# AbnerVictor/OOD-GAN-inversion

Hardware: AMD Instinct MI355X
Metric: 1024² face inversions/sec (100 W+ steps) (higher is better)
Workload: dtype f16-split (hi+lo f16 operands, f32 accumulate): 3 MFMA/product in every forward conv (fp32-equivalent), 2 in the input-gradient convs (back-propagated gradient rounded to f16 before each contraction, weights keep hi+lo); dL/dW+ vs the float64 reference 1.4e-5..3.6e-5 ('f16s': 1.3e-5..2.6e-5, the ref

## Files before the change

include/oodgan.h:

```cpp
#ifndef OODGAN_H
#define OODGAN_H

#ifdef __cplusplus
extern "C" {
#endif

#define OODGAN_OK 0
#define OODGAN_E_ARG (-1)
#define OODGAN_E_LAUNCH (-2)
#define OODGAN_E_STATE (-3)
#define OODGAN_E_NODEV (-4)

int oodgan_version(void);
const char* oodgan_last_error(void);
int oodgan_device_count(void);
int oodgan_set_tunable(const char* name, long value);
long oodgan_get_tunable(const char* name);
long oodgan_dispatch_count(const char* name);
int oodgan_dispatch_reset(void);
int oodgan_zero(void* p, long bytes, void* stream);

void* oodgan_plan_create(void);
int oodgan_plan_destroy(void* plan);
int oodgan_plan_record_begin(void* plan);
// ... 227 lines not shown
int oodgan_reduce_parts(const float* part, float* out, long rows, int nparts, int accumulate, void* stream);
int oodgan_reduce_parts_cols(const float* part, float* out, int B, int C, int nparts, int out_stride, int accumulate,
                             void* stream);


int oodgan_torgb_fwd(const float* x, const float* w, const float* s, int s_stride, const float* bias,
                     const float* skip, const float* kernel, float* y, int B, int Ci, int H, int W,
                     float scale, void* stream);
int oodgan_torgb_fwd_sform(const float* x, const float* w, const float* s, int s_stride, const float* bias,
                           const float* skip, const float* kernel, float* y, void* ys, const float* ys_scale,
                           int ys_scale_stride, int B, int Ci, int H, int W, float scale, unsigned* vmax, void* stream);
int oodgan_rgb_finish(const float* partial, const float* bias, const float* skip, const float* kernel, float* y, int B, int H,
                      int W, void* stream);
int oodgan_rgb_finish_parts(const float* partial, int nparts, const float* bias, const float* skip, const float* kernel, float* y, int B,
                            int H, int W, void* stream);

int oodgan_feature_modulation(const float* x, const float* c0, const float* c1, float* y, long n, int mode, void* stream);

int oodgan_act_bwd_fused(const float* g_feat, const float* out, const float* noise, int noise_batch,
                         const float* noise_w, const float* bias, const float* g_rgb, const float* w_rgb,
                         const float* s_rgb, int s_rgb_stride, float rgb_scale, float* g_pre,
                         float* part_r, float* part_rgb, int B, int C, long HW, void* stream);
int oodgan_act_bwd_nparts(long HW);
int oodgan_act_bwd_fused_max(const float* g_feat, const float* out, const float* noise, int noise_batch,
                             const float* noise_w, const float* bias, const float* g_rgb, const float* w_rgb,
                             const float* s_rgb, int s_rgb_stride, float rgb_scale, float* g_pre,
                             float* part_r, float* part_rgb, float* part_max, const float* dscale, int dscale_stride, int B,
                             int C, long HW, void* stream);
int oodgan_absmax_scale(const float* part, long n, float* out2, void* stream);
int oodgan_absmax_scale_clear(float* part, long n, float* out2, void* stream);
// ... 138 lines not shown
```

ood-gan-inversion_amd/csrc/common.hpp:

```cpp
#pragma once
#include <hip/hip_runtime.h>
#include <cstdio>
#include <cstdarg>
#include <functional>
#include <utility>
#include "../../include/oodgan.h"

namespace oodgan {
struct PlanRec;
extern thread_local PlanRec* tl_plan_rec;
extern int g_null_launch;
void plan_append(std::function<void()>&& f);
template <class F>
inline void launch_rec(F&& f) {
    f();
    if (__builtin_expect(tl_plan_rec != nullptr, 0)) plan_append(std::function<void()>(std::forward<F>(f)));
}
}
#undef hipLaunchKernelGGL
#define hipLaunchKernelGGL(kernelName, numBlocks, numThreads, memPerBlock, streamId, ...)                                        \
    ::oodgan::launch_rec([=]() {                                                                                                 \
        if (!::oodgan::g_null_launch) (kernelName)<<<(numBlocks), (numThreads), (memPerBlock), (streamId)>>>(__VA_ARGS__);      \
    })

namespace oodgan {

void set_error(const char* fmt, ...);

enum { OODGAN_TUN_S1_BIG_MIN_ITEMS = 0, OODGAN_TUN_S2_BIG_MIN_ITEMS, OODGAN_TUN_T2_BIG_MIN_ITEMS, OODGAN_TUN_BLURT_STRIP, OODGAN_TUN_BLUR_STRIP, OODGAN_TUN_UPVB_WAVES, OODGAN_TUN_FEWOUT_QUAD, OODGAN_TUN_TINY_MID_MAX, OODGAN_TUN_STRIPX_WAVES, OODGAN_TUN_BLURT_SEG_ROWS, OODGAN_TUN_COUNT };
long tunable(int id);

enum { OODGAN_DC_STRIPX = 0, OODGAN_DC_STRIP, OODGAN_DC_S1BIG, OODGAN_DC_S1V2, OODGAN_DC_S1PP, OODGAN_DC_TINY, OODGAN_DC_T2BIG,
       OODGAN_DC_T2V2, OODGAN_DC_T2GEN, OODGAN_DC_S2BIG, OODGAN_DC_S2V2, OODGAN_DC_S2GEN, OODGAN_DC_UPVB,
       OODGAN_DC_S1BIG_YS, OODGAN_DC_S2BIG_FUSE, OODGAN_DC_S2BIG_DOTXS,
       OODGAN_DC_S1BIG_G2, OODGAN_DC_S2BIG_G2, OODGAN_DC_STRIPX_G2, OODGAN_DC_S2BIG_XH, OODGAN_DC_S1BIG_XH,
       OODGAN_DC_COMPOSITE_MSE,
       OODGAN_DC_SSIM,
       OODGAN_DC_ROBUST,
       OODGAN_DC_AREA_POOL,
       OODGAN_DC_POOLED_PIXEL,
       OODGAN_DC_PN,
       OODGAN_DC_RESAMPLED_PIXEL,
       OODGAN_DC_BLURT_STRIP, OODGAN_DC_BLURT_TILE, OODGAN_DC_ACTBWD_SFORM, OODGAN_DC_ACTBWD_SFORM_F, OODGAN_DC_COUNT };
void count_dispatch(int id);

bool bound_device_ok(const char* what);

inline int check_launch(const char* what) {
    hipError_t e = hipGetLastError();
    if (e != hipSuccess) {
        set_error("%s: %s", what, hipGetErrorString(e));
        return OODGAN_E_LAUNCH;
    }
    return OODGAN_OK;
}

#define OODGAN_REQUIRE(cond, ...)          \
    do {                                    \
// ... 146 lines not shown
```

ood-gan-inversion_amd/csrc/runtime.hip:

```cpp
#include "common.hpp"
#include <atomic>
#include <cstdlib>
#include <cstring>
#include <new>

namespace oodgan {
static thread_local char g_err[512] = "";
void set_error(const char* fmt, ...) {
    va_list ap;
    va_start(ap, fmt);
    vsnprintf(g_err, sizeof(g_err), fmt, ap);
    va_end(ap);
}
}

namespace oodgan {
namespace {
struct Tunable { const char* name; const char* env; long def; std::atomic<long> val; std::atomic<int> init; };
Tunable g_tun[OODGAN_TUN_COUNT] = {
    {"s1_big_min_items", "OODGAN_S1_BIG_MIN_ITEMS", 128, {0}, {0}},
    {"s2_big_min_items", "OODGAN_S2_BIG_MIN_ITEMS", 128, {0}, {0}},
    {"t2_big_min_items", "OODGAN_T2_BIG_MIN_ITEMS", 128, {0}, {0}},
    {"blurt_strip", "OODGAN_BLURT_STRIP", 1, {0}, {0}},
    {"blur_strip", "OODGAN_BLUR_STRIP", 1, {0}, {0}},
    {"upvb_waves", "OODGAN_UPVB_WAVES", 12, {0}, {0}},
    {"fewout_quad", "OODGAN_FEWOUT_QUAD", 1, {0}, {0}},
    {"tiny_mid_max", "OODGAN_TINY_MID_MAX", 1024, {0}, {0}},
    {"stripx_waves", "OODGAN_STRIPX_WAVES", 4, {0}, {0}},
    {"blurt_seg_rows", "OODGAN_BLURT_SEG_ROWS", 0, {0}, {0}},
};
}
long tunable(int id) {
    Tunable& t = g_tun[id];
    if (!t.init.load(std::memory_order_acquire)) {
        const char* e = getenv(t.env);
        t.val.store(e ? atol(e) : t.def, std::memory_order_relaxed);
        t.init.store(1, std::memory_order_release);
    }
    return t.val.load(std::memory_order_relaxed);
}
}

extern "C" int oodgan_set_tunable(const char* name, long value) {
    OODGAN_REQUIRE(name != nullptr, "set_tunable: null name");
// ... 20 lines not shown
    if (hipGetDevice(&dev) != hipSuccess) {
        (void)hipGetLastError();
        set_error("%s: no current HIP device", what);
        return false;
    }
    int expected = -1;
    if (bound.compare_exchange_strong(expected, dev, std::memory_order_acq_rel) || expected == dev) return true;
    set_error("%s: liboodgan_hip.so is bound to HIP device %d (its first use in this process) but device %d is current — one process per GPU "
              "(select the device with HIP_VISIBLE_DEVICES or torch.cuda.set_device before the first call)", what, expected, dev);
    return false;
}
}

namespace oodgan {
namespace {
const char* const g_dc_name[OODGAN_DC_COUNT] = {"stripx", "strip", "s1big", "s1v2", "s1pp", "tiny", "t2big", "t2v2", "t2gen", "s2big", "s2v2", "s2gen", "upvb", "s1big_ys", "s2big_fuse", "s2big_dotx_sform", "s1big_g2", "s2big_g2", "stripx_g2", "s2big_xh", "s1big_xh", "composite_mse", "ssim", "robust", "area_pool", "pooled_pixel", "pn", "resampled_pixel", "blurt_strip", "blurt_tile", "actbwd_sform", "actbwd_sform_f"};
std::atomic<long> g_dc[OODGAN_DC_COUNT];
}
void count_dispatch(int id) { g_dc[id].fetch_add(1, std::memory_order_relaxed); }
}
extern "C" long oodgan_dispatch_count(const char* name) {
    if (name)
        for (int i = 0; i < oodgan::OODGAN_DC_COUNT; ++i)
            if (strcmp(name, oodgan::g_dc_name[i]) == 0) return oodgan::g_dc[i].load(std::memory_order_relaxed);
    return -1;
}
extern "C" int oodgan_dispatch_reset(void) {
    for (int i = 0; i < oodgan::OODGAN_DC_COUNT; ++i) oodgan::g_dc[i].store(0, std::memory_order_relaxed);
    return OODGAN_OK;
}

// ... 85 lines not shown
```

ood-gan-inversion_amd/oodgan/_lib.py:

```python
import ctypes
import os
from ctypes import POINTER, Structure, c_char_p, c_double, c_float, c_int, c_long, c_void_p

_HERE = os.path.dirname(os.path.abspath(__file__))
LIB_PATH = os.environ.get('OODGAN_LIB') or os.path.join(_HERE, 'liboodgan_hip.so')

CONV_S1, CONV_T2, CONV_S2 = 0, 1, 2
ACT_NONE, ACT_LRELU, ACT_PRELU = 0, 1, 2

P = c_void_p


ABI_VERSION = 117


class ConvArgs(Structure):
    _fields_ = [
        ('x', P), ('wpk', P), ('in_scale', P), ('in_shift', P), ('out_scale', P), ('bias', P), ('noise', P),
        ('noise_w', P), ('slope', P), ('dotx', P), ('dot_part', P), ('y', P),
        ('B', c_int), ('K', c_int), ('M', c_int), ('Hin', c_int), ('Win', c_int),
        ('in_pitch', c_int), ('out_pitch', c_int), ('in_scale_stride', c_int), ('out_scale_stride', c_int),
        ('noise_batch', c_int), ('mode', c_int), ('act', c_int), ('dot_nparts', c_int), ('in_mul2', P),
        ('x_sform', c_int), ('ys', P), ('ys_scale', P), ('ys_scale_stride', c_int),
        ('rgb_w', P), ('rgb_s', P), ('rgb_y', P), ('rgb_s_stride', c_int), ('rgb_scale', c_float), ('fuse', P), ('dot_actgrad', c_int), ('groups', c_int), ('y_fform', c_int), ('x_fform', c_int), ('dotx_fform', c_int), ('dotx_sform', c_int), ('dotx_scale', P), ('dotx_scale_stride', c_int), ('workspace', P), ('workspace_bytes', c_long), ('ys_vmax', P), ('x_hi_only', c_int),
# ... 95 lines not shown
    'oodgan_demod_bwd_batch': (c_int, [P, c_int, P]),
    'oodgan_demod_fwd_batch': (c_int, [P, c_int, P]),
    'oodgan_absmax_scale_check_batch': (c_int, [P, c_int, P, P]),
    'oodgan_hform_bytes': (c_long, [c_int, c_int, c_int, c_int]),
    'oodgan_to_hform': (c_int, [P, P, c_int, c_int, c_int, c_int, P]),
    'oodgan_from_hform': (c_int, [P, P, c_int, c_int, c_int, c_int, P]),
    'oodgan_modconv_f16_wbytes': (c_long, [c_int, c_int, c_int]),
    'oodgan_modconv_f16_pack': (c_int, [P, P, c_int, c_float, c_int, c_int, P, c_int, c_int, c_int, P]),
    'oodgan_modconv_f16_pack_affine': (c_int, [P, P, c_int, P, P, c_int, c_float, c_int, c_int, P, c_int, c_int, c_int, P]),
    'oodgan_modconv_f16': (c_int, [P, P, P, c_int, P, P, c_int, P, c_int, c_int, c_int, c_int, c_int, P]),
    'oodgan_reduce_parts': (c_int, [P, P, c_long, c_int, c_int, P]),
    'oodgan_reduce_parts_cols': (c_int, [P, P, c_int, c_int, c_int, c_int, c_int, P]),
    'oodgan_torgb_fwd': (c_int, [P, P, P, c_int, P, P, P, P, c_int, c_int, c_int, c_int, c_float, P]),
    'oodgan_rgb_finish': (c_int, [P, P, P, P, P, c_int, c_int, c_int, P]),
    'oodgan_rgb_finish_parts': (c_int, [P, c_int, P, P, P, P, c_int, c_int, c_int, P]),
    'oodgan_torgb_fwd_sform': (c_int, [P, P, P, c_int, P, P, P, P, P, P, c_int, c_int, c_int, c_int, c_int, c_float, P, P]),
    'oodgan_act_bwd_fused': (c_int, [P, P, P, c_int, P, P, P, P, P, c_int, c_float, P, P, P, c_int, c_int, c_long, P]),
    'oodgan_act_bwd_nparts': (c_int, [c_long]),
    'oodgan_feature_modulation': (c_int, [P, P, P, P, c_long, c_int, P]),
    'oodgan_act_bwd_fused_max': (c_int, [P, P, P, c_int, P, P, P, P, P, c_int, c_float, P, P, P, P, P, c_int, c_int, c_int, c_long, P]),
    'oodgan_absmax_scale': (c_int, [P, c_long, P, P]),
    'oodgan_absmax_scale_clear': (c_int, [P, c_long, P, P]),
    'oodgan_mse_fwd_bwd': (c_int, [P, P, P, P, P, c_int, c_long, c_float, P]),
    'oodgan_mse_fwd_bwd_row': (c_int, [P, P, P, P, P, P, c_int, c_int, c_long, c_float, P]),
    'oodgan_conv2d_s1': (c_int, [P, P, P, P, P, P, c_int, c_int, c_int, c_int, c_int, c_int, c_int, c_int, P]),
    'oodgan_add_mask': (c_int, [P, P, P, c_long, P]),
    'oodgan_maxpool3s2_fwd': (c_int, [P, P, P, c_long, c_int, c_int, P]),
    'oodgan_maxpool3s2_bwd': (c_int, [P, P, P, P, P, c_long, c_int, c_int, P]),
    'oodgan_lpips_prep': (c_int, [P, P, c_int, c_int, c_int, c_float, c_float, POINTER(c_float), POINTER(c_float), P]),
    'oodgan_lpips_img_grad': (c_int, [P, P, c_int, c_int, c_int, c_float, c_float, POINTER(c_float), P]),
# ... 117 lines not shown
```

ood-gan-inversion_amd/oodgan/engine.py:

```python
import math
import numbers
import re

import os

import torch

from . import ops
from ._lib import ACT_LRELU, ACT_NONE, CONV_S1, CONV_S2, CONV_T2
from .synth import generator_channels, make_kernel


_Cols = ops.Cols


class _Layer:
    __slots__ = ('name', 'kind', 'cin', 'cout', 'res', 'lat', 'row', 'drow', 'wpk', 'wpk_bwd', 'wsq', 'w_rgb',
                 'bias', 'noise_w', 'scale', 'noise_idx', 'src', 'sidx', 'wpk_vb')


def _pad_channels_to_16(state, prefix, log_size, ch):
    up16 = lambda c: (c + 15) // 16 * 16
    chp = {r: up16(c) for r, c in ch.items()}
    out = dict(state)
# ... 242 lines not shown
    def style_layout(self):
        if self.padded:
            raise NotImplementedError('style_layout() of a generator whose channel counts are zero-padded to multiples of 16')
        lay = style_layout(self.log_size, lambda name: self.by_name[name].cin)
        assert lay == [(L.name, L.lat, L.row, L.cin) for L in self.layers]
        return lay

    def feature_shape(self, l):
        l = check_feature_layer(l, self.n_latent)
        if self.padded:
            raise NotImplementedError('feature_layer on a generator whose channel counts are zero-padded to multiples of 16')
        L = next(L for L in self.layers if L.kind == 'up' and L.lat == l)
        return (L.cin, L.res // 2, L.res // 2)

    def forward(self, latent, noises, save=False, cond_hook=None, cond_layers=None, return_features=False, features_in=None,
                feature_scale=1.0, range_mode='exact', post_hook=None, style_offsets=None, feature_offset=None, feature_out=None):
        if self.padded and (cond_hook is not None or features_in is not None or post_hook is not None):
            raise NotImplementedError('conditioning hooks / feature injection on a generator whose channel counts are zero-padded to multiples of 16')
        if save and (features_in is not None or post_hook is not None):
            raise NotImplementedError('backward through an injected feature / feature modulation is not part of the path')
        if self.padded and style_offsets is not None:
            raise NotImplementedError('style offsets on a generator whose channel counts are zero-padded to multiples of 16')
        B = latent.shape[0]
        f_lat, f_delta, f_in = None, None, None
        if feature_offset is not None:
            f_lat, f_delta = feature_offset
            if tuple(f_delta.shape) != (B,) + self.feature_shape(f_lat):
                raise ValueError(f'feature_offset for latent {f_lat} must be {(B,) + self.feature_shape(f_lat)}, got {tuple(f_delta.shape)}')
        self._fwd_serial += 1
        s_all = self.styles(latent, style_offsets)
        d_all = torch.empty(B, self.DR, device=self.device, dtype=torch.float32)
# ... 26 lines not shown
                                vmax=rng.vm[L.sidx] if carry else None)

        acts = {}
        ck = (B, ops._stream_handle())
        x = self._const_b.get(ck)
        if x is None:
            x = self._const_b[ck] = self.const_input.expand(B, -1, -1, -1).contiguous()
        acts['input'] = x
        skip, out = None, x
        pending = None
        rgb_partial = None
        i = 1
        for L in self.layers:
            s = _Cols(s_all, L.row, L.cin)
            if L.kind == 'rgb' and rgb_partial is not None:
                skip = ops.rgb_finish(rgb_partial, L.bias, skip, self.k_up if skip is not None else None)
                rgb_partial = None
                continue
            if L.kind == 'rgb':
                Lu = self.rgb_next_up.get(L.name) if (carry and self.fused_rgb) else None
                if (Lu is not None and pending is None and out.shape[2] * out.shape[3] > 4096 and L.cin % 16 == 0
                        and out.shape[3] % 4 == 0):
                    pending = ops.sform_scratch(B, L.cin, out.shape[2], out.shape[3], self.device)
                    skip = ops.torgb(out, L.w_rgb, s, L.bias, skip, self.k_up if skip is not None else None, ys=pending,
                                     ys_scale=_Cols(s_use, Lu.row, Lu.cin), vmax=rng.vm[Lu.sidx])
                else:
                    skip = ops.torgb(out, L.w_rgb, s, L.bias, skip, self.k_up if skip is not None else None)
                continue
            d = _Cols(d_use, L.drow, L.cout)
            nz = noises[L.noise_idx]
            if features_in is not None and L.lat >= 1 and L.lat < len(features_in) and features_in[L.lat] is not None:
# ... 118 lines not shown
            return skip, (feat[:, :self.real_channels[self.size]].contiguous() if self.padded else feat)
        return skip

    def _demod(self, L, s_all, d_all):
        from ._lib import lib, check
        import ctypes
        B = s_all.shape[0]
        check(lib().oodgan_demod_fwd(ctypes.c_void_p(s_all.data_ptr() + 4 * L.row), self.R, ctypes.c_void_p(L.wsq.data_ptr()),
                                     ctypes.c_void_p(d_all.data_ptr() + 4 * L.drow), self.DR, B, L.cin, L.cout, L.scale,
                                     ops._stream()), 'demod_fwd')

    def _hi_records(self, B, L, Hd, Rg):
        return bool(self.grad_hi_only and self.hi_records and Rg is None and ops.blurT_hi_supported(Hd, Hd)
                    and ops.s2_fuse_supported(B, L.cout, L.cin, 2 * Hd + 1, 2 * Hd + 1))

    def backward(self, gimg, grad_scale=1.0, carry_scale=False, wrt='latent', feature_grad=None):
        from ._lib import lib, check
        import ctypes
        if wrt not in ('latent', 'styles'):
            raise ValueError(f"wrt must be 'latent' or 'styles', got {wrt!r}")
        sv = self.saved
        if sv is None:
            raise RuntimeError('backward() without forward(save=True)')
        if sv['serial'] != self._fwd_serial:
            raise RuntimeError('backward(): another forward of this engine ran after forward(save=True) — the saved activations (pooled S-form / F-form '
                               'buffers, scales of the range state) may have been overwritten; call backward() right after the forward it belongs to')
        acts, s_all, d_all, noises, B = sv['acts'], sv['s_all'], sv['d_all'], sv['noises'], sv['B']
        f_lat, f_in = sv['f_lat'], sv['f_in']
        if (feature_grad is not None) != (f_lat is not None):
            raise RuntimeError('backward(feature_grad=) goes with forward(feature_offset=, save=True), and one needs the other')
        if feature_grad is not None and not (tuple(feature_grad.shape) == tuple(f_in.shape) and feature_grad.dtype == torch.float32
                                             and feature_grad.is_contiguous() and feature_grad.device == f_in.device):
            raise ValueError(f'feature_grad must be a contiguous float32 {tuple(f_in.shape)} tensor on {f_in.device}')
        gs_all = ops.zeros(B, self.R, device=self.device)
        gskip = {self.size: gimg.contiguous()}
        r = self.size
        while r > 4:
            gskip[r // 2] = ops.upfirdn2d(gskip[r], self.k_up_flip, up=1, down=2, pad=(1, 1))
            r //= 2
        g_feat = None
        prev_rgb = None
        fused_in = None
        fused_pre = None
        jobs = ops.BwdJobs() if (carry_scale and self.fused_bwd and self.sform and self.batched_tail) else None
        for L in reversed(self.layers):
            if L.kind == 'rgb':
                prev_rgb = L
                continue
            out, x_in, nz = acts[L.name], acts[L.src], noises[L.noise_idx]
            at_f = L.lat == f_lat
            if at_f:
# ... 153 lines not shown
        return torch.cuda.MemPool()
    key = (str(device), ops._stream_handle(), int(batch))
    pool = _PLAN_POOLS.get(key)
    if pool is None:
        pool = _PLAN_POOLS[key] = torch.cuda.MemPool()
    return pool


def _flag_stream(device):
    st = _FLAG.get(str(device))
    if st is None:
        st = _FLAG[str(device)] = torch.cuda.Stream(device=device)
    return st


class _WRun:

    def __init__(self, inv, eng, target, w0, noises, steps, stream, keep_traj, replay, beta=None, ids=None, anchor=None, f0=None, pn=None,
                 px=None, ml0=None):
        self.inv, self.eng, self.stream, self.steps = inv, eng, stream, steps
        self.target, self.noises = target, noises
        self.beta = beta
        self.sspace = inv.latent_space == 's'
        self.w0 = w0.detach().clone().contiguous() if self.sspace else None
        self.w = torch.zeros(w0.shape[0], eng.R, device=w0.device, dtype=torch.float32) if self.sspace else w0.detach().clone().contiguous()
        self.m, self.v = torch.zeros_like(self.w), torch.zeros_like(self.w)
        self.gmul = ops.loss_scale_for(target.numel() // target.shape[0])
        self.t = 0
        self.dev_t = torch.zeros(1, dtype=torch.int32, device=self.w.device)
        self.lbuf = torch.empty(steps, self.w.shape[0], device=self.w.device, dtype=torch.float32)
# ... 25 lines not shown
            self.fm, self.fv, self.fg, self.fx = (torch.zeros_like(self.f) for _ in range(4))
            if inv.feature_reg != 0.0:
                self.ft_table = torch.zeros(steps, self.w.shape[0], device=self.w.device, dtype=torch.float32)
                self.fpart = ops.feature_step_parts(self.f.shape[0], self.f.numel() // self.f.shape[0], self.f.device)
        self.pn = pn
        self.pn_table = torch.zeros(steps, self.w.shape[0], device=self.w.device, dtype=torch.float32) if inv.pn_reg != 0.0 else None
        self.pn_part = ops.pn_prior_parts(self.w.shape[0], self.w.shape[1], self.w.device) if self.pn_table is not None else None
        self.ml = self.mm = self.mv = self.mg = self.ma = self.me = self.mstat = self.ma_table = self.mb_table = None
        if ml0 is not None:
            Bm, S = self.w.shape[0], int(target.shape[-1])
            self.ml = ml0.detach().clone().contiguous()
            self.mm, self.mv, self.mg, self.ma = (torch.zeros_like(self.ml) for _ in range(4))
            self.beta, self.me = (torch.empty(Bm, 1, S, S, device=self.w.device, dtype=torch.float32) for _ in range(2))
            self.mstat = ops.maskfit_stat(Bm, self.w.device)
            self.ma_table, self.mb_table = (torch.zeros(steps, Bm, device=self.w.device, dtype=torch.float32) for _ in range(2))
        self.traj = [None] * steps if keep_traj else None
        self.mode0 = (eng.fused_bwd, eng.carry_range)
        self.guard = (eng.fused_bwd or eng.carry_range) and inv.check_every > 0 and replay != 'graph'
        self.clean = (0, self.w.clone(), None, None, self._fsnap(), self._msnap()) if self.guard else None
        self.pending, self.exact_until = None, 0
        self.steps_run = 0
        self.rollbacks = 0
        self.host = inv._pinned(len(inv._runs)) if self.guard else None
        inv._runs.append(self)
        if replay == 'plan' and (keep_traj or not eng.sform):
            replay = None
        self.replay, self.warmup = replay, 1 if replay == 'graph' else 2
        self.plan, self.pool, self.eager_left, self.plan_steps, self.plan_size = None, None, self.warmup, 0, 0

    def _eager_step(self):
# ... 7 lines not shown
                           style_reg=inv.style_reg, table=self.st_table)
            return
        w_in = self.w
        if self.w_in is not None:
            w_in = ops.latent_noise(self.w, self.dev_t, self.ids, self.steps, inv.latent_noise, inv.noise_ramp, inv.noise_seed, out=self.w_in,
                                    period=self.w.shape[-1] if self.tied else None)
        if self.ml is not None:
            ops.maskfit_expand(self.ml, int(self.target.shape[-1]), a=self.ma, beta=self.beta)
            img = eng.forward(w_in, self.noises, save=True, range_mode='carry')
            gimg = self._loss_grad(img)
            g = eng.backward(gimg, self.gmul, carry_scale=True)
            ops.maskfit_step(self.ml, self.mg, self.mm, self.mv, self.ma, self.me, self.dev_t, self.steps, inv.lr_rampup, inv.lr_rampdown,
                             inv.mask_lr, inv.betas, inv.eps, grad_div=self.gmul, area=inv.mask_area, area_weight=inv.mask_area_weight,
                             binary_weight=inv.mask_binary_weight, area_table=self.ma_table, binary_table=self.mb_table, stat=self.mstat)
        elif self.f is None:
            img = eng.forward(w_in, self.noises, save=True, range_mode='carry')
            gimg = self._loss_grad(img)
            g = eng.backward(gimg, self.gmul, carry_scale=True)
        else:
            img = eng.forward(w_in, self.noises, save=True, range_mode='carry', feature_offset=(inv.feature_layer, self.f), feature_out=self.fx)
            gimg = self._loss_grad(img)
            g = eng.backward(gimg, self.gmul, carry_scale=True, feature_grad=self.fg)
            ops.feature_step(self.f, self.fg, self.fm, self.fv, self.dev_t, self.steps, inv.lr_rampup, inv.lr_rampdown, inv.feature_lr,
                             inv.betas, inv.eps, grad_div=self.gmul, feature_reg=inv.feature_reg, table=self.ft_table, part=self.fpart)
        if self.lat_table is not None:
            ops.latent_prior_loss_grad(self.w, self.anchor, g, inv.latent_reg, table=self.lat_table, row_dev=self.dev_t)
        if self.pn_table is not None:
            ops.pn_prior_loss_grad(self.w, self.pn.mean, self.pn.matrix, g, inv.pn_reg, table=self.pn_table, row_dev=self.dev_t, part=self.pn_part)
        if self.controls:
            ops.latent_step(self.w, g, self.m, self.v, self.dev_t, self.steps, inv.lr_rampup, inv.lr_rampdown, inv.lr, inv.betas, inv.eps,
                            layer_lr=self.layer_lr, delta_reg=inv.delta_reg, tied=self.tied, table=self.dl_table)
        elif inv.lr_rampup > 0.0 or inv.lr_rampdown > 0.0:
            ops.adam_step_dev_sched(self.w, g, self.m, self.v, self.dev_t, self.steps, inv.lr_rampup, inv.lr_rampdown, inv.lr, inv.betas, inv.eps)
        else:
            ops.adam_step_dev(self.w, g, self.m, self.v, self.dev_t, inv.lr, inv.betas, inv.eps)

    def _loss_grad(self, img):
        inv, gmul, row = self.inv, self.gmul, self.dev_t
        fit = self.ml is not None
        on_c = self.beta is not None and (self.lp is not None or self.ss_table is not None)
        _, gimg, c = ops.pixel_loss_grad(img, self.target, inv.pixel_loss, inv.pixel_scale, self.beta, gmul, wrt='composite' if (on_c or fit) else 'gen',
                                         composite=on_c, table=self.lbuf, row_dev=row, pool=self.px_f, target_pooled=self.px_target,
                                         resample=self.px_tables)
        x = c if on_c else img
        if self.lp is not None and self.lp_f == 1:
            self.lp.loss_and_grad(x, gimg, inv.lpips_weight * gmul, table=self.lp_table, row_dev=row, target_taps=self.lp_target)
        elif self.lp is not None:
            xs, gs = ops.area_pool(x, self.lp_f, grad_buffer=True)
            self.lp.loss_and_grad(xs, gs, inv.lpips_weight * gmul, table=self.lp_table, row_dev=row, target_taps=self.lp_target)
            ops.area_pool_bwd_add(gs, gimg, self.lp_f)
        if self.ss_table is not None:
            ops.ssim_loss_grad(x, self.target, gimg, inv.ssim_weight * gmul, table=self.ss_table, row_dev=row)
        if fit:
# ... 633 lines not shown
```

ood-gan-inversion_amd/oodgan/ops.py:

```python
import ctypes
import os
import math

import torch

from . import _lib
from ._lib import ACT_LRELU, ACT_NONE, ACT_PRELU, CONV_S1, CONV_S2, CONV_T2, ConvArgs, check

SQRT2 = 2 ** 0.5


def _p(t):
    return None if t is None else ctypes.c_void_p(t.data_ptr())


_RAW_STREAM = getattr(torch._C, '_cuda_getCurrentRawStream', None)
_DEV_INDEX = None


def _stream_handle():
    global _DEV_INDEX
    if _RAW_STREAM is None:
        return torch.cuda.current_stream().cuda_stream
    if _DEV_INDEX is None:
# ... 967 lines not shown
            self.t = _reduce_parts(self.part_t, B * C, self.nparts)


def rgb_finish(partial, bias=None, skip=None, kernel=None):
    if partial.dim() == 5:
        n, B, _, H, W = partial.shape
        check(_lib.lib().oodgan_rgb_finish_parts(_p(partial), n, _p(_opt(bias, 'bias')), _p(_opt(skip, 'skip')), _p(_opt(kernel, 'kernel')),
                                                 _p(partial), B, H, W, _stream()), 'rgb_finish_parts')
        return partial[0]
    B, _, H, W = partial.shape
    check(_lib.lib().oodgan_rgb_finish(_p(partial), _p(_opt(bias, 'bias')), _p(_opt(skip, 'skip')), _p(_opt(kernel, 'kernel')),
                                       _p(partial), B, H, W, _stream()), 'rgb_finish')
    return partial


def torgb(x, weight, s, bias=None, skip=None, kernel=None, ys=None, ys_scale=None, vmax=None):
    x = _dev(x)
    B, Ci, H, W = x.shape
    y = torch.empty(B, 3, H, W, device=x.device, dtype=torch.float32)
    w = _dev(weight, 'weight').reshape(3, Ci)
    if ys is not None:
        check(_lib.lib().oodgan_torgb_fwd_sform(_p(x), _p(w), _p(_dev(s, 's')), s.shape[1], _p(_opt(bias, 'bias')), _p(_opt(skip, 'skip')),
                                                _p(_opt(kernel, 'kernel')), _p(y), _p(ys), _p(_opt(ys_scale, 'ys_scale')),
                                                0 if ys_scale is None else ys_scale.shape[1], B, Ci, H, W, 1.0 / math.sqrt(Ci),
                                                _p(vmax), _stream()), 'torgb_fwd_sform')
        return y
    check(_lib.lib().oodgan_torgb_fwd(_p(x), _p(w), _p(_dev(s, 's')), s.shape[1], _p(_opt(bias, 'bias')), _p(_opt(skip, 'skip')),
                                      _p(_opt(kernel, 'kernel')), _p(y), B, Ci, H, W, 1.0 / math.sqrt(Ci), _stream()), 'torgb_fwd')
    return y

# ... 626 lines not shown
```

Baseline: 8.144.

## Fuse final RGB finish, MSE loss/grad and first skip downsample into one kernel

Adds a fused image-tail kernel that sums the ToRGB partials, adds bias and the upsampled skip, computes the MSE loss and gradient, and produces the half-resolution skip gradient. This avoids materialising the image and re-reading it for the loss and the first down-filter. It also adds a single-launch down2 pyramid kernel for the small skip-gradient levels, replacing a chain of upfirdn2d launches. The fused path needs band-halo recomputation and shape restrictions, and is enabled by default only for plain MSE runs.

```diff
diff --git a/include/oodgan.h b/include/oodgan.h
--- a/include/oodgan.h
+++ b/include/oodgan.h
@@ -265,6 +265,12 @@
                       int W, void* stream);
 int oodgan_rgb_finish_parts(const float* partial, int nparts, const float* bias, const float* skip, const float* kernel, float* y, int B,
                             int H, int W, void* stream);
+
+int oodgan_image_tail_supported(int C, int H, int W);
+int oodgan_image_tail_mse(const float* partial, int nparts, const float* bias, const float* skip, const float* kernel, const float* target,
+                          const float* kernel_flip, float* gimg, float* gskip, float* img, float* part, float* loss_table,
+                          const int* row_dev, int nrows, int B, int C, int H, int W, float grad_mul, void* stream);
+int oodgan_down2_pyramid(const float* x, const float* kernel_flip, float* const* levels, int nlevels, int planes, int n, void* stream);
 
 int oodgan_feature_modulation(const float* x, const float* c0, const float* c1, float* y, long n, int mode, void* stream);
 
diff --git a/ood-gan-inversion_amd/csrc/common.hpp b/ood-gan-inversion_amd/csrc/common.hpp
--- a/ood-gan-inversion_amd/csrc/common.hpp
+++ b/ood-gan-inversion_amd/csrc/common.hpp
@@ -27,7 +27,7 @@
 
 void set_error(const char* fmt, ...);
 
-enum { OODGAN_TUN_S1_BIG_MIN_ITEMS = 0, OODGAN_TUN_S2_BIG_MIN_ITEMS, OODGAN_TUN_T2_BIG_MIN_ITEMS, OODGAN_TUN_BLURT_STRIP, OODGAN_TUN_BLUR_STRIP, OODGAN_TUN_UPVB_WAVES, OODGAN_TUN_FEWOUT_QUAD, OODGAN_TUN_TINY_MID_MAX, OODGAN_TUN_STRIPX_WAVES, OODGAN_TUN_BLURT_SEG_ROWS, OODGAN_TUN_COUNT };
+enum { OODGAN_TUN_S1_BIG_MIN_ITEMS = 0, OODGAN_TUN_S2_BIG_MIN_ITEMS, OODGAN_TUN_T2_BIG_MIN_ITEMS, OODGAN_TUN_BLURT_STRIP, OODGAN_TUN_BLUR_STRIP, OODGAN_TUN_UPVB_WAVES, OODGAN_TUN_FEWOUT_QUAD, OODGAN_TUN_TINY_MID_MAX, OODGAN_TUN_STRIPX_WAVES, OODGAN_TUN_BLURT_SEG_ROWS, OODGAN_TUN_IMG_TAIL_FUSED, OODGAN_TUN_COUNT };
 long tunable(int id);
 
 enum { OODGAN_DC_STRIPX = 0, OODGAN_DC_STRIP, OODGAN_DC_S1BIG, OODGAN_DC_S1V2, OODGAN_DC_S1PP, OODGAN_DC_TINY, OODGAN_DC_T2BIG,
@@ -41,7 +41,8 @@
        OODGAN_DC_POOLED_PIXEL,
        OODGAN_DC_PN,
        OODGAN_DC_RESAMPLED_PIXEL,
-       OODGAN_DC_BLURT_STRIP, OODGAN_DC_BLURT_TILE, OODGAN_DC_ACTBWD_SFORM, OODGAN_DC_ACTBWD_SFORM_F, OODGAN_DC_COUNT };
+       OODGAN_DC_BLURT_STRIP, OODGAN_DC_BLURT_TILE, OODGAN_DC_ACTBWD_SFORM, OODGAN_DC_ACTBWD_SFORM_F,
+       OODGAN_DC_IMG_TAIL, OODGAN_DC_DOWN2_PYR, OODGAN_DC_COUNT };
 void count_dispatch(int id);
 
 bool bound_device_ok(const char* what);
diff --git a/ood-gan-inversion_amd/csrc/image_tail.hip b/ood-gan-inversion_amd/csrc/image_tail.hip
--- /dev/null
+++ b/ood-gan-inversion_amd/csrc/image_tail.hip
@@ -0,0 +1,302 @@
+#include "loss_common.hpp"
+
+using namespace oodgan;
+
+namespace {
+
+constexpr int kTailThreads = 256;
+constexpr int kChunk4 = kMseChunk / 4;
+constexpr int kPerThread = kChunk4 / kTailThreads;
+constexpr int kBatch = 2;
+
+__device__ __forceinline__ float from_left(float v) { return __shfl_up(v, 1, 64); }
+__device__ __forceinline__ float from_right(float v) { return __shfl_down(v, 1, 64); }
+
+struct TailArgs {
+    const float* part;
+    const float* bias;
+    const float* skip;
+    const float* target;
+    float* gimg;
+    float* gskip;
+    float* img;
+    float* lpart;
+    int nparts, B, H, W;
+    float gscale;
+};
+
+template <int NP>
+struct TailPx {
+    float4 p[NP > 0 ? NP : 1], t;
+    float sv[2][4];
+
+    __device__ __forceinline__ void load(const TailArgs& a, long pl, int Y, int X) {
+        const long HW = (long)a.H * a.W;
+        const long e = (long)Y * a.W + X;
+        const float* pp = a.part + pl * HW + e;
+#pragma unroll
+        for (int q = 0; q < (NP > 0 ? NP : 1); ++q) p[q] = ld4_stream(pp + (long)q * a.B * 3 * HW);
+        t = ld4_stream(a.target + pl * HW + e);
+        if (a.skip) {
+            const int h2 = a.H >> 1, w2 = a.W >> 1, x2 = X >> 1;
+            const float* sp = a.skip + pl * h2 * w2;
+#pragma unroll
+            for (int u = 0; u < 2; ++u) {
+                const int ky = (Y & 1) + 2 * u;
+                const int iy = (Y + ky - 2) >> 1;
+                const float* rp = sp + (long)min(max(iy, 0), h2 - 1) * w2;
+                const float2 m = *reinterpret_cast<const float2*>(rp + x2);
+                sv[u][0] = rp[max(x2 - 1, 0)];
+                sv[u][1] = m.x;
+                sv[u][2] = m.y;
+                sv[u][3] = rp[min(x2 + 2, w2 - 1)];
+            }
+        }
+    }
+
+    __device__ __forceinline__ float4 finish(const TailArgs& a, const float* __restrict__ kf, long pl, int c, int Y, int X) const {
+        float4 o = p[0];
+#pragma unroll
+        for (int q = 1; q < NP; ++q) { o.x += p[q].x; o.y += p[q].y; o.z += p[q].z; o.w += p[q].w; }
+        if constexpr (NP == 0) {
+            const long HW = (long)a.H * a.W;
+            const float* pp = a.part + pl * HW + (long)Y * a.W + X;
+            for (int q = 1; q < a.nparts; ++q) {
+                const float4 v = *reinterpret_cast<const float4*>(pp + (long)q * a.B * 3 * HW);
+                o.x += v.x; o.y += v.y; o.z += v.z; o.w += v.w;
+            }
+        }
+        if (a.bias) {
+            const float bv = a.bias[c];
+            o.x += bv; o.y += bv; o.z += bv; o.w += bv;
+        }
+        if (a.skip) {
+            const int h2 = a.H >> 1, w2 = a.W >> 1;
+            float r[4] = {o.x, o.y, o.z, o.w};
+#pragma unroll
+            for (int j = 0; j < 4; ++j) {
+#pragma unroll
+                for (int u = 0; u < 2; ++u) {
+                    const int ky = (Y & 1) + 2 * u;
+                    const int iy = (Y + ky - 2) >> 1;
+                    const bool yok = Y + ky - 2 >= 0 && iy < h2;
+#pragma unroll
+                    for (int v = 0; v < 2; ++v) {
+                        const int kx = (j & 1) + 2 * v;
+                        const int ix = (X + j + kx - 2) >> 1;
+                        const bool ok = yok && X + j + kx - 2 >= 0 && ix < w2;
+                        const float w = ok ? kf[ky * 4 + kx] : 0.f;
+                        if (w != 0.f) r[j] += w * sv[u][(j + kx) >> 1];
+                    }
+                }
+            }
+            o = make_float4(r[0], r[1], r[2], r[3]);
+        }
+        return o;
+    }
+};
+
+template <int NP>
+__global__ __launch_bounds__(kTailThreads, 6) void image_tail_mse_kernel(const TailArgs a, const float* __restrict__ kern,
+                                                                      const float* __restrict__ kflip) {
+    extern __shared__ __attribute__((aligned(16))) float gl[];
+    __shared__ float kf[16], kd[16], red[4];
+    const int tid = threadIdx.x;
+    if (tid < 16) {
+        kf[tid] = a.skip ? kern[(3 - tid / 4) * 4 + (3 - tid % 4)] : 0.f;
+        kd[tid] = kflip[15 - tid];
+    }
+    __syncthreads();
+    const int W = a.W, H = a.H, W4 = W >> 2, sh = __ffs(W4) - 1, R = kMseChunk >> (sh + 2);
+    const int band = blockIdx.x, c = blockIdx.y, b = blockIdx.z;
+    const long pl = (long)b * 3 + c;
+    const long HW = (long)H * W;
+    const int r0 = band * R;
+    float* gp = a.gimg + pl * HW;
+    float* ip = a.img ? a.img + pl * HW : nullptr;
+    const float gscale = a.gscale;
+
+    float acc = 0.f;
+#pragma unroll 1
+    for (int k0 = 0; k0 < kPerThread; k0 += kBatch) {
+        TailPx<NP> px[kBatch];
+#pragma unroll
+        for (int u = 0; u < kBatch; ++u) {
+            const int i = tid + kTailThreads * (k0 + u);
+            px[u].load(a, pl, r0 + (i >> sh), 4 * (i & (W4 - 1)));
+        }
+#pragma unroll
+        for (int u = 0; u < kBatch; ++u) {
+            const int i = tid + kTailThreads * (k0 + u);
+            const int Y = r0 + (i >> sh), X = 4 * (i & (W4 - 1));
+            const float4 o = px[u].finish(a, kf, pl, c, Y, X);
+            const float4 t = px[u].t;
+            const float4 d = make_float4(o.x - t.x, o.y - t.y, o.z - t.z, o.w - t.w);
+            float4 psi;
+            const float rx = rho_psi<kSquare>(d.x, 0.f, 0.f, psi.x), ry = rho_psi<kSquare>(d.y, 0.f, 0.f, psi.y);
+            const float rz = rho_psi<kSquare>(d.z, 0.f, 0.f, psi.z), rw = rho_psi<kSquare>(d.w, 0.f, 0.f, psi.w);
+            const float4 g = make_float4(psi.x * gscale, psi.y * gscale, psi.z * gscale, psi.w * gscale);
+            acc += rx + ry + rz + rw;
+            const long e = (long)Y * W + X;
+            *reinterpret_cast<float4*>(gp + e) = g;
+            if (ip) st4_stream(ip + e, o);
+        }
+    }
+    for (int j = tid; j < 2 * W4; j += kTailThreads) {
+        const bool top = j < W4;
+        const int Y = top ? r0 - 1 : r0 + R, X = 4 * (top ? j : j - W4);
+        float4 g = make_float4(0.f, 0.f, 0.f, 0.f);
+        if (Y >= 0 && Y < H) {
+            TailPx<NP> px;
+            px.load(a, pl, Y, X);
+            const float4 o = px.finish(a, kf, pl, c, Y, X);
+            const float4 d = make_float4(o.x - px.t.x, o.y - px.t.y, o.z - px.t.z, o.w - px.t.w);
+            g = make_float4(d.x * gscale, d.y * gscale, d.z * gscale, d.w * gscale);
+        }
+        *reinterpret_cast<float4*>(gl + (top ? 0 : W) + X) = g;
+    }
+    acc = block_sum_256(acc, red);
+    if (tid == 0) a.lpart[(long)b * (3 * (HW / kMseChunk)) + c * (HW / kMseChunk) + band] = acc;
+
+    const int h2 = H >> 1, w2 = W >> 1, lane = tid & 63;
+    float* sp = a.gskip + pl * h2 * w2;
+    const int items = (R >> 1) * W4;
+    for (int n = tid; n < items; n += kTailThreads) {
+        const int orow = n >> sh, og = n & (W4 - 1);
+        const int oy = (r0 >> 1) + orow;
+        const bool first = orow == 0, last = orow == (R >> 1) - 1;
+        const bool lf_own = lane == 0 || og == 0, rt_own = lane == 63 || og == W4 - 1;
+        const int cl = max(4 * og - 1, 0), cr = min(4 * og + 4, W - 1);
+        float4 m[4];
+        float lf[4], rt[4];
+#pragma unroll
+        for (int ky = 0; ky < 4; ++ky) {
+            const int iy = min(max(2 * oy - 1 + ky, r0), r0 + R - 1);
+            const float* rp = gp + (long)iy * W;
+            m[ky] = *reinterpret_cast<const float4*>(rp + 4 * og);
+            lf[ky] = lf_own ? rp[cl] : 0.f;
+            rt[ky] = rt_own ? rp[cr] : 0.f;
+        }
+        if (first) {
+            m[0] = *reinterpret_cast<const float4*>(gl + 4 * og);
+            lf[0] = gl[cl];
+            rt[0] = gl[cr];
+        }
+        if (last) {
+            m[3] = *reinterpret_cast<const float4*>(gl + W + 4 * og);
+            lf[3] = gl[W + cl];
+            rt[3] = gl[W + cr];
+        }
+        float acc0 = 0.f, acc1 = 0.f;
+#pragma unroll
+        for (int ky = 0; ky < 4; ++ky) {
+            const float l = from_left(m[ky].w), r = from_right(m[ky].x);
+            const int iy = 2 * oy - 1 + ky;
+            const bool yok = iy >= 0 && iy < H;
+            const float v[6] = {lf_own ? lf[ky] : l, m[ky].x, m[ky].y, m[ky].z, m[ky].w, rt_own ? rt[ky] : r};
+#pragma unroll
+            for (int kx = 0; kx < 4; ++kx) {
+                const int ix0 = 4 * og - 1 + kx, ix1 = ix0 + 2;
+                if (yok && ix0 >= 0 && ix0 < W) acc0 += kd[ky * 4 + kx] * v[kx];
+                if (yok && ix1 >= 0 && ix1 < W) acc1 += kd[ky * 4 + kx] * v[kx + 2];
+            }
+        }
+        *reinterpret_cast<float2*>(sp + (long)oy * w2 + 2 * og) = make_float2(acc0, acc1);
+    }
+}
+
+struct PyrArgs {
+    const float* x;
+    float* y[16];
+    int n, levels;
+};
+
+__global__ __launch_bounds__(1024) void down2_pyramid_kernel(const PyrArgs a, const float* __restrict__ kflip) {
+    __shared__ float kf[16];
+    if (threadIdx.x < 16) kf[threadIdx.x] = kflip[15 - threadIdx.x];
+    __syncthreads();
+    const long pl = blockIdx.x;
+    int in = a.n;
+    const float* xp = a.x + pl * in * in;
+    for (int l = 0; l < a.levels; ++l) {
+        const int on = in >> 1;
+        float* yp = a.y[l] + pl * on * on;
+        for (int e = threadIdx.x; e < on * on; e += 1024) {
+            const int ox = e % on, oy = e / on;
+            const int y0 = 2 * oy - 1, x0 = 2 * ox - 1;
+            float v[16];
+#pragma unroll
+            for (int ky = 0; ky < 4; ++ky)
+#pragma unroll
+                for (int kx = 0; kx < 4; ++kx) v[ky * 4 + kx] = xp[min(max(y0 + ky, 0), in - 1) * in + min(max(x0 + kx, 0), in - 1)];
+            float acc = 0.f;
+#pragma unroll
+            for (int ky = 0; ky < 4; ++ky)
+#pragma unroll
+                for (int kx = 0; kx < 4; ++kx) {
+                    const int iy = y0 + ky, ix = x0 + kx;
+                    if (iy >= 0 && iy < in && ix >= 0 && ix < in) acc += kf[ky * 4 + kx] * v[ky * 4 + kx];
+                }
+            yp[oy * on + ox] = acc;
+        }
+        __threadfence_block();
+        __syncthreads();
+        xp = yp;
+        in = on;
+    }
+}
+
+}
+
+extern "C" int oodgan_image_tail_supported(int C, int H, int W) {
+    if (C != 3 || H <= 0 || W <= 0 || (H & 1)) return 0;
+    if (W < 8 || kMseChunk % W != 0 || ((kMseChunk / W) & 1)) return 0;
+    if (((long)H * W) % kMseChunk != 0) return 0;
+    if (W > 4096) return 0;
+    return 1;
+}
+
+extern "C" int oodgan_image_tail_mse(const float* partial, int nparts, const float* bias, const float* skip, const float* kernel,
+                                     const float* target, const float* kernel_flip, float* gimg, float* gskip, float* img, float* part,
+                                     float* loss_table, const int* row_dev, int nrows, int B, int C, int H, int W, float grad_mul,
+                                     void* stream) {
+    OODGAN_REQUIRE(partial && target && kernel_flip && gimg && gskip && part && loss_table && nparts >= 1 && B > 0 && B <= 65535,
+                   "image_tail_mse: bad args");
+    OODGAN_REQUIRE(!row_dev || nrows > 0, "image_tail_mse: a row needs nrows > 0");
+    OODGAN_REQUIRE(!skip || kernel, "image_tail_mse: skip needs kernel");
+    OODGAN_REQUIRE(oodgan_image_tail_supported(C, H, W),
+                   "image_tail_mse: shape (%d, %d, %d): needs C = 3, H even, 16384 %% W == 0 with an even quotient, H*W %% 16384 == 0", C, H, W);
+    OODGAN_REQUIRE(img != partial, "image_tail_mse: the image cannot be written over the partial sums (bands read their neighbours' rows)");
+    const long CHW = 3L * H * W;
+    const int lds = 2 * W * 4;
+    TailArgs a{partial, bias, skip, target, gimg, gskip, img, part, nparts, B, H, W, grad_mul * 2.0f / (float)CHW};
+    const dim3 grid((unsigned)((long)H * W / kMseChunk), 3, B);
+    count_dispatch(OODGAN_DC_IMG_TAIL);
+    if (nparts == 1)
+        hipLaunchKernelGGL(image_tail_mse_kernel<1>, grid, dim3(kTailThreads), lds, as_stream(stream), a, kernel, kernel_flip);
+    else if (nparts == 2)
+        hipLaunchKernelGGL(image_tail_mse_kernel<2>, grid, dim3(kTailThreads), lds, as_stream(stream), a, kernel, kernel_flip);
+    else
+        hipLaunchKernelGGL(image_tail_mse_kernel<0>, grid, dim3(kTailThreads), lds, as_stream(stream), a, kernel, kernel_flip);
+    int rc = check_launch("image_tail_mse");
+    if (rc != OODGAN_OK) return rc;
+    hipLaunchKernelGGL(mean_finish_kernel<>, dim3(B), dim3(64), 0, as_stream(stream), part, loss_table, oodgan_mse_nparts(CHW),
+                       1.0f / (float)CHW, row_dev, row_dev ? nrows : 1);
+    return check_launch("image_tail_mse_finish");
+}
+
+extern "C" int oodgan_down2_pyramid(const float* x, const float* kernel_flip, float* const* levels, int nlevels, int planes, int n,
+                                    void* stream) {
+    OODGAN_REQUIRE(x && kernel_flip && levels && planes > 0, "down2_pyramid: bad args");
+    OODGAN_REQUIRE(n >= 8 && (n & (n - 1)) == 0 && n <= 4096, "down2_pyramid: size %d: a power of two from 8 to 4096", n);
+    OODGAN_REQUIRE(nlevels >= 1 && nlevels <= 16 && (n >> nlevels) >= 1, "down2_pyramid: %d levels below %d", nlevels, n);
+    PyrArgs a{};
+    a.x = x; a.n = n; a.levels = nlevels;
+    for (int l = 0; l < nlevels; ++l) {
+        OODGAN_REQUIRE(levels[l] != nullptr, "down2_pyramid: level %d is null", l);
+        a.y[l] = levels[l];
+    }
+    count_dispatch(OODGAN_DC_DOWN2_PYR);
+    hipLaunchKernelGGL(down2_pyramid_kernel, dim3(planes), dim3(1024), 0, as_stream(stream), a, kernel_flip);
+    return check_launch("down2_pyramid");
+}
diff --git a/ood-gan-inversion_amd/csrc/runtime.hip b/ood-gan-inversion_amd/csrc/runtime.hip
--- a/ood-gan-inversion_amd/csrc/runtime.hip
+++ b/ood-gan-inversion_amd/csrc/runtime.hip
@@ -28,6 +28,7 @@
     {"tiny_mid_max", "OODGAN_TINY_MID_MAX", 1024, {0}, {0}},
     {"stripx_waves", "OODGAN_STRIPX_WAVES", 4, {0}, {0}},
     {"blurt_seg_rows", "OODGAN_BLURT_SEG_ROWS", 0, {0}, {0}},
+    {"img_tail_fused", "OODGAN_IMG_TAIL_FUSED", 1, {0}, {0}},
 };
 }
 long tunable(int id) {
@@ -78,7 +79,7 @@
 
 namespace oodgan {
 namespace {
-const char* const g_dc_name[OODGAN_DC_COUNT] = {"stripx", "strip", "s1big", "s1v2", "s1pp", "tiny", "t2big", "t2v2", "t2gen", "s2big", "s2v2", "s2gen", "upvb", "s1big_ys", "s2big_fuse", "s2big_dotx_sform", "s1big_g2", "s2big_g2", "stripx_g2", "s2big_xh", "s1big_xh", "composite_mse", "ssim", "robust", "area_pool", "pooled_pixel", "pn", "resampled_pixel", "blurt_strip", "blurt_tile", "actbwd_sform", "actbwd_sform_f"};
+const char* const g_dc_name[OODGAN_DC_COUNT] = {"stripx", "strip", "s1big", "s1v2", "s1pp", "tiny", "t2big", "t2v2", "t2gen", "s2big", "s2v2", "s2gen", "upvb", "s1big_ys", "s2big_fuse", "s2big_dotx_sform", "s1big_g2", "s2big_g2", "stripx_g2", "s2big_xh", "s1big_xh", "composite_mse", "ssim", "robust", "area_pool", "pooled_pixel", "pn", "resampled_pixel", "blurt_strip", "blurt_tile", "actbwd_sform", "actbwd_sform_f", "img_tail", "down2_pyr"};
 std::atomic<long> g_dc[OODGAN_DC_COUNT];
 }
 void count_dispatch(int id) { g_dc[id].fetch_add(1, std::memory_order_relaxed); }
diff --git a/ood-gan-inversion_amd/oodgan/_lib.py b/ood-gan-inversion_amd/oodgan/_lib.py
--- a/ood-gan-inversion_amd/oodgan/_lib.py
+++ b/ood-gan-inversion_amd/oodgan/_lib.py
@@ -133,6 +133,9 @@
     'oodgan_torgb_fwd': (c_int, [P, P, P, c_int, P, P, P, P, c_int, c_int, c_int, c_int, c_float, P]),
     'oodgan_rgb_finish': (c_int, [P, P, P, P, P, c_int, c_int, c_int, P]),
     'oodgan_rgb_finish_parts': (c_int, [P, c_int, P, P, P, P, c_int, c_int, c_int, P]),
+    'oodgan_image_tail_supported': (c_int, [c_int, c_int, c_int]),
+    'oodgan_image_tail_mse': (c_int, [P, c_int, P, P, P, P, P, P, P, P, P, P, P, c_int, c_int, c_int, c_int, c_int, c_float, P]),
+    'oodgan_down2_pyramid': (c_int, [P, P, P, c_int, c_int, c_int, P]),
     'oodgan_torgb_fwd_sform': (c_int, [P, P, P, c_int, P, P, P, P, P, P, c_int, c_int, c_int, c_int, c_int, c_float, P, P]),
     'oodgan_act_bwd_fused': (c_int, [P, P, P, c_int, P, P, P, P, P, c_int, c_float, P, P, P, c_int, c_int, c_long, P]),
     'oodgan_act_bwd_nparts': (c_int, [c_long]),
diff --git a/ood-gan-inversion_amd/oodgan/engine.py b/ood-gan-inversion_amd/oodgan/engine.py
--- a/ood-gan-inversion_amd/oodgan/engine.py
+++ b/ood-gan-inversion_amd/oodgan/engine.py
@@ -280,7 +280,7 @@
         return (L.cin, L.res // 2, L.res // 2)
 
     def forward(self, latent, noises, save=False, cond_hook=None, cond_layers=None, return_features=False, features_in=None,
-                feature_scale=1.0, range_mode='exact', post_hook=None, style_offsets=None, feature_offset=None, feature_out=None):
+                feature_scale=1.0, range_mode='exact', post_hook=None, style_offsets=None, feature_offset=None, feature_out=None, defer_tail=False):
         if self.padded and (cond_hook is not None or features_in is not None or post_hook is not None):
             raise NotImplementedError('conditioning hooks / feature injection on a generator whose channel counts are zero-padded to multiples of 16')
         if save and (features_in is not None or post_hook is not None):
@@ -337,7 +337,11 @@
         for L in self.layers:
             s = _Cols(s_all, L.row, L.cin)
             if L.kind == 'rgb' and rgb_partial is not None:
-                skip = ops.rgb_finish(rgb_partial, L.bias, skip, self.k_up if skip is not None else None)
+                if (defer_tail and L is self.layers[-1] and not return_features
+                        and ops.image_tail_supported(3, rgb_partial.shape[-2], rgb_partial.shape[-1])):
+                    skip = ops.RgbTail(rgb_partial, L.bias, skip, self.k_up if skip is not None else None)
+                else:
+                    skip = ops.rgb_finish(rgb_partial, L.bias, skip, self.k_up if skip is not None else None)
                 rgb_partial = None
                 continue
             if L.kind == 'rgb':
@@ -486,7 +490,7 @@
         return bool(self.grad_hi_only and self.hi_records and Rg is None and ops.blurT_hi_supported(Hd, Hd)
                     and ops.s2_fuse_supported(B, L.cout, L.cin, 2 * Hd + 1, 2 * Hd + 1))
 
-    def backward(self, gimg, grad_scale=1.0, carry_scale=False, wrt='latent', feature_grad=None):
+    def backward(self, gimg, grad_scale=1.0, carry_scale=False, wrt='latent', feature_grad=None, gskip_half=None):
         from ._lib import lib, check
         import ctypes
         if wrt not in ('latent', 'styles'):
@@ -507,6 +511,16 @@
         gs_all = ops.zeros(B, self.R, device=self.device)
         gskip = {self.size: gimg.contiguous()}
         r = self.size
+        if gskip_half is not None:
+            gskip[r // 2] = gskip_half
+            r //= 2
+            while r > max(4, PYRAMID_FROM):
+                gskip[r // 2] = ops.upfirdn2d(gskip[r], self.k_up_flip, up=1, down=2, pad=(1, 1))
+                r //= 2
+            if r > 4:
+                for t in ops.down2_pyramid(gskip[r], self.k_up_flip):
+                    gskip[t.shape[-1]] = t
+                r = 4
         while r > 4:
             gskip[r // 2] = ops.upfirdn2d(gskip[r], self.k_up_flip, up=1, down=2, pad=(1, 1))
             r //= 2
@@ -690,6 +704,9 @@
     return st
 
 
+PYRAMID_FROM = 128
+
+
 class _WRun:
 
     def __init__(self, inv, eng, target, w0, noises, steps, stream, keep_traj, replay, beta=None, ids=None, anchor=None, f0=None, pn=None,
@@ -745,6 +762,10 @@
             self.beta, self.me = (torch.empty(Bm, 1, S, S, device=self.w.device, dtype=torch.float32) for _ in range(2))
             self.mstat = ops.maskfit_stat(Bm, self.w.device)
             self.ma_table, self.mb_table = (torch.zeros(steps, Bm, device=self.w.device, dtype=torch.float32) for _ in range(2))
+        self.tail_fused = (ops.image_tail_fused() and inv.pixel_loss == 'mse' and beta is None and ml0 is None and self.px_f == 1
+                           and inv.pixel_filter is None and self.lp is None and self.ss_table is None and not self.sspace and self.f is None
+                           and tuple(target.shape[1:]) == (3, eng.size, eng.size))
+        self.gskip_half = None
         self.traj = [None] * steps if keep_traj else None
         self.mode0 = (eng.fused_bwd, eng.carry_range)
         self.guard = (eng.fused_bwd or eng.carry_range) and inv.check_every > 0 and replay != 'graph'
@@ -782,9 +803,10 @@
                              inv.mask_lr, inv.betas, inv.eps, grad_div=self.gmul, area=inv.mask_area, area_weight=inv.mask_area_weight,
                              binary_weight=inv.mask_binary_weight, area_table=self.ma_table, binary_table=self.mb_table, stat=self.mstat)
         elif self.f is None:
-            img = eng.forward(w_in, self.noises, save=True, range_mode='carry')
+            img = eng.forward(w_in, self.noises, save=True, range_mode='carry', defer_tail=self.tail_fused and inv.on_step is None)
             gimg = self._loss_grad(img)
-            g = eng.backward(gimg, self.gmul, carry_scale=True)
+            half, self.gskip_half = self.gskip_half, None
+            g = eng.backward(gimg, self.gmul, carry_scale=True, **({} if half is None else dict(gskip_half=half)))
         else:
             img = eng.forward(w_in, self.noises, save=True, range_mode='carry', feature_offset=(inv.feature_layer, self.f), feature_out=self.fx)
             gimg = self._loss_grad(img)
@@ -805,6 +827,10 @@
 
     def _loss_grad(self, img):
         inv, gmul, row = self.inv, self.gmul, self.dev_t
+        if isinstance(img, ops.RgbTail):
+            _, gimg, self.gskip_half, _ = ops.image_tail_mse(img.partial, img.bias, img.skip, img.kernel, self.target, self.eng.k_up_flip, gmul,
+                                                             table=self.lbuf, row_dev=row)
+            return gimg
         fit = self.ml is not None
         on_c = self.beta is not None and (self.lp is not None or self.ss_table is not None)
         _, gimg, c = ops.pixel_loss_grad(img, self.target, inv.pixel_loss, inv.pixel_scale, self.beta, gmul, wrt='composite' if (on_c or fit) else 'gen',
diff --git a/ood-gan-inversion_amd/oodgan/ops.py b/ood-gan-inversion_amd/oodgan/ops.py
--- a/ood-gan-inversion_amd/oodgan/ops.py
+++ b/ood-gan-inversion_amd/oodgan/ops.py
@@ -1005,6 +1005,62 @@
     return partial
 
 
+class RgbTail:
+
+    def __init__(self, partial, bias, skip, kernel):
+        self.partial, self.bias, self.skip, self.kernel = partial, bias, skip, kernel
+        self.shape = (partial.shape[-4], 3, partial.shape[-2], partial.shape[-1])
+
+    def finish(self):
+        return rgb_finish(self.partial, self.bias, self.skip, self.kernel)
+
+
+def image_tail_fused():
+    return _lib.lib().oodgan_get_tunable(b'img_tail_fused') != 0
+
+
+def image_tail_supported(C, H, W):
+    return bool(_lib.lib().oodgan_image_tail_supported(int(C), int(H), int(W)))
+
+
+def image_tail_mse(partial, bias, skip, kernel, target, kernel_flip, grad_mul=1.0, loss_out=None, table=None, row_dev=None, want_img=False):
+    part5 = _dev(partial, 'partial')
+    n = part5.shape[0] if part5.dim() == 5 else 1
+    B, C, H, W = part5.shape[-4:]
+    t = _dev(target, 'target')
+    if tuple(t.shape) != (B, C, H, W):
+        raise ValueError(f'target must be {(B, C, H, W)}, got {tuple(t.shape)}')
+    sk = _opt(skip, 'skip')
+    if sk is not None and tuple(sk.shape) != (B, C, H // 2, W // 2):
+        raise ValueError(f'skip must be {(B, C, H // 2, W // 2)}, got {tuple(sk.shape)}')
+    L = _lib.lib()
+    g = torch.empty(B, C, H, W, device=t.device, dtype=torch.float32)
+    gs = torch.empty(B, C, H // 2, W // 2, device=t.device, dtype=torch.float32)
+    img = torch.empty(B, C, H, W, device=t.device, dtype=torch.float32) if want_img else None
+    part = torch.empty(B, L.oodgan_mse_nparts(C * H * W), device=t.device, dtype=torch.float32)
+    dst, row, nrows, by_row, loss = _loss_sink(B, t.device, loss_out, table, row_dev)
+    check(L.oodgan_image_tail_mse(_p(part5), n, _p(_opt(bias, 'bias')), _p(sk), _p(_opt(kernel, 'kernel')), _p(t), _p(_dev(kernel_flip, 'kernel_flip')),
+                                  _p(g), _p(gs), _p(img), _p(part), _p(dst), _p(row), nrows, B, C, H, W, float(grad_mul), _stream()),
+          'image_tail_mse')
+    return loss, g, gs, img
+
+
+def down2_pyramid(x, kernel_flip, nlevels=None):
+    x = _dev(x)
+    B, C, n, n2 = x.shape
+    if n != n2:
+        raise ValueError(f'down2_pyramid: square planes, got {tuple(x.shape)}')
+    if nlevels is None:
+        nlevels = max(0, int(n).bit_length() - 3)
+    sizes = [n >> (l + 1) for l in range(nlevels)]
+    out = [torch.empty(B, C, s, s, device=x.device, dtype=torch.float32) for s in sizes]
+    if not out:
+        return out
+    ptrs = (ctypes.c_void_p * nlevels)(*[t.data_ptr() for t in out])
+    check(_lib.lib().oodgan_down2_pyramid(_p(x), _p(_dev(kernel_flip, 'kernel_flip')), ptrs, nlevels, B * C, n, _stream()), 'down2_pyramid')
+    return out
+
+
 def torgb(x, weight, s, bias=None, skip=None, kernel=None, ys=None, ys_scale=None, vmax=None):
     x = _dev(x)
     B, Ci, H, W = x.shape
```

After: 8.030. -1.4%, worse.
